# EEA-sensors/parallel-gps

Hardware: AMD Instinct MI355X
Metric: timesteps/sec (filter+smooth+log-lik) (higher is better)
Workload: dtype f64; 1 GPU; c2: matern32 state-dim 2, N=2^20 steps per GPU (1048576 total), f64, irregular times, prior-sampled observations; steps_per_gpu=1048576, steps_total=1048576, state_dim=2, parallelism=1 GPU

## Files before the change

### parallel-gps_amd/csrc/pgps_core.hip

```cpp
#include <chrono>
#include <algorithm>
#include <cmath>
#include <cstdlib>
#include <vector>
#include <cstdio>
#include <cstring>
#include <new>

#include "pgps_internal.h"
#include "pgps_gradlti.h"
#include "pgps_wc_args.h"

using namespace pgps;

namespace pgps {
int ensure(pgps_ctx* ctx, DevBuf& b, size_t bytes) {
    if (&b == &ctx->ws) ++ctx->ws_epoch;
    if (bytes <= b.cap) return PGPS_OK;
    if (b.p) HIPCHK(ctx, hipFree(b.p));
    b.p = nullptr;
    b.cap = 0;
    size_t want = bytes + bytes / 8 + 256;
    hipError_t e = hipMalloc(&b.p, want);
    if (e != hipSuccess) {
// ... 1048 lines not shown
template <typename T>
static int seg_smoother(pgps_ctx* ctx, long N, int d, int rank, int nranks, const T* Fs, const T* Qs, const T* fms,
                        const T* fPs, const T* gathered_s, T* sms, T* sPs, double* ll) {
    ScanArgs<T> a{};
    TRY(seg_common<T>(ctx, N, d, rank, nranks, a));
    if (!Fs || !Qs || !fms || !fPs || !gathered_s || !sms || !sPs) return PGPS_E_INVALID;
    if (!aligned16(Fs) || !aligned16(Qs) || !aligned16(fms) || !aligned16(fPs) || !aligned16(sms) ||
        !aligned16(sPs) || !aligned16(gathered_s))
        return PGPS_E_INVALID;
    a.Fs = Fs; a.Qs = Qs; a.fms = const_cast<T*>(fms); a.fPs = const_cast<T*>(fPs);
    a.gathered_s = gathered_s; a.sms = sms; a.sPs = sPs; a.ll = ll;
    if (!seg_follows(ctx, 3, N, d, rank, nranks)) return PGPS_E_INVALID;
    ctx->seg_tag.phase = 0;
    return dispatch_scan<T>(ctx, d, a, MODE_SEG_SMOOTHER);
}

#define PGPS_DEFINE_SEG(SUF, T)                                                                                      \
    extern "C" int pgps_seg_filter_reduce_dev_##SUF(pgps_ctx* c, long N, int d, int rank, int nranks, const T* P0,   \
                                                    const T* Fs, const T* Qs, const T* H, T R, const T* ys,         \
                                                    T* rec_f) {                                                     \
        return seg_reduce<T>(c, N, d, rank, nranks, P0, Fs, Qs, H, R, ys, rec_f);                                   \
    }                                                                                                                \
    extern "C" int pgps_seg_filter_apply_dev_##SUF(pgps_ctx* c, long N, int d, int rank, int nranks, const T* P0,    \
                                                   const T* Fs, const T* Qs, const T* H, T R, const T* ys,          \
                                                   const T* gathered_f, T* fms, T* fPs, T* rec_s) {                 \
        return seg_filter<T>(c, N, d, rank, nranks, P0, Fs, Qs, H, R, ys, gathered_f, fms, fPs, rec_s);             \
    }                                                                                                                \
    extern "C" int pgps_seg_smoother_apply_dev_##SUF(pgps_ctx* c, long N, int d, int rank, int nranks, const T* Fs,  \
                                                     const T* Qs, const T* fms, const T* fPs, const T* gathered_s,  \
                                                     T* sms, T* sPs, double* ll) {                                  \
        return seg_smoother<T>(c, N, d, rank, nranks, Fs, Qs, fms, fPs, gathered_s, sms, sPs, ll);                  \
    }

PGPS_DEFINE_SEG(f64, double)
PGPS_DEFINE_SEG(f32, float)

template <typename T>
static int pkfs_seg_run(pgps_ctx* ctx, long N, int d, const T* P0, const T* Fs, const T* Qs, const T* H, T R, const T* ys,
                        T* fms, T* fPs, T* sms, T* sPs, double* ll) {
    RoctxRange range_("parallel_filter");
    const int rank = ctx->comm_rank, nranks = ctx->comm_nranks;
    const size_t rf = ((size_t)seg_rec_f_len(d) * sizeof(T) + 15) / 16 * 16, rs = ((size_t)seg_rec_s_len(d) * sizeof(T) + 15) / 16 * 16;
    TRY(ensure(ctx, ctx->comm_buf, (rf + rs) * (size_t)(nranks + 1)));
    char* base = (char*)ctx->comm_buf.p;
    T* rec_f = (T*)base;
    T* rec_s = (T*)(base + rf);
    T* gat_f = (T*)(base + rf + rs);
    T* gat_s = (T*)(base + rf + rs + rf * (size_t)nranks);
    TRY(seg_reduce<T>(ctx, N, d, rank, nranks, P0, Fs, Qs, H, R, ys, rec_f));
    TRY(comm_allgather(ctx, rec_f, gat_f, (size_t)seg_rec_f_len(d) * sizeof(T)));
    TRY(seg_filter<T>(ctx, N, d, rank, nranks, P0, Fs, Qs, H, R, ys, gat_f, fms, fPs, rec_s));
    TRY(comm_allgather(ctx, rec_s, gat_s, (size_t)seg_rec_s_len(d) * sizeof(T)));
    return seg_smoother<T>(ctx, N, d, rank, nranks, Fs, Qs, fms, fPs, gat_s, sms, sPs, ll);
}

template <typename T>
static int pkfs_seg_dev(pgps_ctx* ctx, long N, int d, const T* P0, const T* Fs, const T* Qs, const T* H, T R, const T* ys,
                        T* fms, T* fPs, T* sms, T* sPs, double* ll) {
    if (!ctx || N < 1 || !P0 || !Fs || !Qs || !H || !ys || !fms || !fPs || !sms || !sPs) return PGPS_E_INVALID;
    if (!ctx->comm) return PGPS_E_INVALID;
    if (d < 1 || d > PGPS_MAX_DIM) return PGPS_E_UNSUPPORTED_DIM;
    return pkfs_seg_run<T>(ctx, N, d, P0, Fs, Qs, H, R, ys, fms, fPs, sms, sPs, ll);
}

extern "C" int pgps_pkfs_seg_dev_f64(pgps_ctx* c, long N, int d, const double* P0, const double* Fs, const double* Qs,
                                     const double* H, double R, const double* ys, double* fms, double* fPs, double* sms,
                                     double* sPs, double* ll) {
    return pkfs_seg_dev<double>(c, N, d, P0, Fs, Qs, H, R, ys, fms, fPs, sms, sPs, ll);
}
extern "C" int pgps_pkfs_seg_dev_f32(pgps_ctx* c, long N, int d, const float* P0, const float* Fs, const float* Qs,
                                     const float* H, float R, const float* ys, float* fms, float* fPs, float* sms, float* sPs,
                                     double* ll) {
    return pkfs_seg_dev<float>(c, N, d, P0, Fs, Qs, H, R, ys, fms, fPs, sms, sPs, ll);
}

template <typename T>
static int gp_dev(pgps_ctx* ctx, long N, int d, double lam, const double* N1, const double* N2, const double* Pinf,
                  const double* H, double R, const T* ts, double t0, const T* ys, T* fms, T* fPs, T* sms, T* sPs,
                  double* ll) {
    RoctxRange range_("parallel_filter");
    if (!ctx || N < 1 || !N1 || !Pinf || !H || !ts || !ys) return PGPS_E_INVALID;
    if (d < 1 || d > 3) return PGPS_E_UNSUPPORTED_DIM;
    if ((fms == nullptr) != (fPs == nullptr) || (sms == nullptr) != (sPs == nullptr)) return PGPS_E_INVALID;
    if (sms && !fms) return PGPS_E_INVALID;
    if (!fms && !ll) return PGPS_E_INVALID;
    if ((fms && (!aligned16(fms) || !aligned16(fPs))) || (sms && (!aligned16(sms) || !aligned16(sPs))))
        return PGPS_E_INVALID;
    GpArgs<T> g{};
    g.s.N = N;
    g.s.R = (T)R;
    g.s.ys = ys;
    g.s.fms = fms; g.s.fPs = fPs; g.s.sms = sms; g.s.sPs = sPs; g.s.ll = ll;
    g.m.lam = lam;
    for (int i = 0; i < 9; ++i) { g.m.N1[i] = 0; g.m.N2[i] = 0; g.m.Pinf[i] = 0; }
    for (int i = 0; i < d * d; ++i) { g.m.N1[i] = N1[i]; g.m.N2[i] = N2 ? N2[i] : 0.0; g.m.Pinf[i] = Pinf[i]; }
    for (int i = 0; i < 3; ++i) g.m.H[i] = i < d ? (T)H[i] : T(0);
    g.m.ts = ts;
    g.m.t_prev = (T)t0;
    if constexpr (sizeof(T) == 8) {
        if (resident_fits(ctx, N, d, false) && aligned16(ts) && aligned16(ys)) {
            ResArgs<double> ra{};
            ra.s = g.s;
            ra.m = g.m;
            return launch_resident<double, 2>(ctx, ra, true, sms != nullptr);
        }
    }
    switch (d) {
        case 1: return launch_gp<T, 1>(ctx, g, fms != nullptr, sms != nullptr);
        case 2: return launch_gp<T, 2>(ctx, g, fms != nullptr, sms != nullptr);
        case 3: return launch_gp<T, 3>(ctx, g, fms != nullptr, sms != nullptr);
        default: return PGPS_E_UNSUPPORTED_DIM;
    }
}

static int gp_adj_dev(pgps_ctx* ctx, long N, int d, double lam, const double* N1, const double* N2, const double* Pinf,
                      const double* H, double R, const double* ts, double t0, const double* ys, double* out) {
    RoctxRange range_("parallel_filter");
    if (!ctx || N < 1 || !N1 || !Pinf || !H || !ts || !ys || !out) return PGPS_E_INVALID;
    if (d < 1 || d > 3) return PGPS_E_UNSUPPORTED_DIM;
    GpArgs<double> g{};
    g.s.N = N;
    g.s.R = R;
    g.s.ys = ys;
    g.m.lam = lam;
    for (int i = 0; i < 9; ++i) { g.m.N1[i] = 0; g.m.N2[i] = 0; g.m.Pinf[i] = 0; }
    for (int i = 0; i < d * d; ++i) { g.m.N1[i] = N1[i]; g.m.N2[i] = N2 ? N2[i] : 0.0; g.m.Pinf[i] = Pinf[i]; }
    for (int i = 0; i < 3; ++i) g.m.H[i] = i < d ? H[i] : 0.0;
    g.m.ts = ts;
    g.m.t_prev = t0;
    switch (d) {
        case 1: return launch_gp_adj<double, 1>(ctx, g, out);
        case 2: return launch_gp_adj<double, 2>(ctx, g, out);
        case 3: return launch_gp_adj<double, 3>(ctx, g, out);
        default: return PGPS_E_UNSUPPORTED_DIM;
    }
}

extern "C" int pgps_gp_ll_grad_adj_dev_f64(pgps_ctx* ctx, long N, int d, double lam, const double* N1, const double* N2,
                                           const double* Pinf, const double* H, double R, const double* ts, double t0,
                                           const double* ys, double* out) {
    return gp_adj_dev(ctx, N, d, lam, N1, N2, Pinf, H, R, ts, t0, ys, out);
}

template <typename T>
static int gp_host(pgps_ctx* ctx, long N, int d, double lam, const double* N1, const double* N2, const double* Pinf,
                   const double* H, double R, const T* ts, double t0, const T* ys, T* fms, T* fPs, T* sms, T* sPs,
                   double* ll) {
    if (!ctx || N < 1 || !ts || !ys) return PGPS_E_INVALID;
    if (d < 1 || d > 3) return PGPS_E_UNSUPPORTED_DIM;
    HIPCHK(ctx, hipSetDevice(ctx->device));
    const size_t n = (size_t)N, dd = (size_t)d * d;
    const bool wf = fms || fPs || sms || sPs, wsm = sms || sPs;
    if (!wf) {
        SmallStage st(ctx, 2 * SmallStage::up(n * sizeof(T)), 16);
        if (st.ok) {
            double llh = 0.0;
            T* dys_ = st.in(ys, n);
            T* dts_ = st.in(ts, n);
            double* dll_ = st.out(&llh, 1);
            TRY(st.send());
            TRY(gp_dev<T>(ctx, N, d, lam, N1, N2, Pinf, H, R, dts_, t0, dys_, nullptr, nullptr, nullptr, nullptr, dll_));
            TRY(st.finish());
            if (ll) *ll = llh;
            return std::isfinite(llh) ? PGPS_OK : PGPS_E_NUMERIC;
        }
    }
    T *dts, *dys, *dfms = nullptr, *dfPs = nullptr, *dsms = nullptr, *dsPs = nullptr;
    double* dll;
    TRY(stage_in(ctx, ctx->st[4], ys, n, &dys));
    TRY(stage_in(ctx, ctx->st[10], ts, n, &dts));
    if (wf) {
        TRY(stage_in<T>(ctx, ctx->st[5], nullptr, n * d, &dfms));
        TRY(stage_in<T>(ctx, ctx->st[6], nullptr, n * dd, &dfPs));
    }
    if (wsm) {
        TRY(stage_in<T>(ctx, ctx->st[7], nullptr, n * d, &dsms));
        TRY(stage_in<T>(ctx, ctx->st[8], nullptr, n * dd, &dsPs));
    }
    TRY(stage_in<double>(ctx, ctx->st[9], nullptr, 2, &dll));
    TRY(gp_dev<T>(ctx, N, d, lam, N1, N2, Pinf, H, R, dts, t0, dys, dfms, dfPs, dsms, dsPs, dll));
    if (fms) TRY(stage_out(ctx, fms, dfms, n * d));
    if (fPs) TRY(stage_out(ctx, fPs, dfPs, n * dd));
    if (sms) TRY(stage_out(ctx, sms, dsms, n * d));
    if (sPs) TRY(stage_out(ctx, sPs, dsPs, n * dd));
    double llh = 0.0;
    TRY(stage_out(ctx, &llh, dll, 1));
    HIPCHK(ctx, hipStreamSynchronize(ctx->stream));
    if (ll) *ll = llh;
    if (!std::isfinite(llh)) return PGPS_E_NUMERIC;
// ... 1775 lines not shown
```

### parallel-gps_amd/csrc/pgps_resident.hip.h

```cpp
#pragma once

#include <type_traits>

#include "pgps_fused.hip.h"
#include "pgps_kernels.hip.h"

namespace pgps {


template <typename T, int D, int LC>
struct ResCfg {
    static constexpr int W = (int)sizeof(T), MAT = D * D, G = 4;
    static_assert(LC % G == 0, "whole sub-tiles");
    static constexpr int S = LC / G;
    using GF = StageGeom<MAT * W, G>;
    using GM = StageGeom<D * W, G>;
    static constexpr int SLOT = LC * MAT * W + 16;
    static constexpr int SLOTS = kWave * SLOT;
    static constexpr int MST = GM::BYTES > 5120 ? GM::BYTES : 5120;
    static constexpr int NSCAN = kWaves * Dim<D>::NFILT * W;
    static constexpr int BYTES = kWaves * (SLOTS + MST) + NSCAN + kWaves * 8;
};

__device__ __forceinline__ void res_wave_sync() {
    __builtin_amdgcn_fence(__ATOMIC_RELEASE, "wavefront");
    __builtin_amdgcn_wave_barrier();
    __builtin_amdgcn_fence(__ATOMIC_ACQUIRE, "wavefront");
}

template <typename T> struct ResForget;
template <> struct ResForget<double> { static constexpr double kA = 0x1p-120; };
template <> struct ResForget<float> { static constexpr float kA = 0x1p-60f; };

#define PGPS_RSTAMP(IDX)                                                                              \
    do {                                                                                              \
        if (ra.stamps && threadIdx.x == 0) ra.stamps[(long)blockIdx.x * 16 + (IDX)] = __builtin_readcyclecounter(); \
    } while (0)
#define PGPS_RSTAMP_WAVE(K)                                                                           \
    do {                                                                                              \
        if (ra.stamps && lane == 0)                                                                   \
            ra.stamps[(long)gridDim.x * 16 + (long)blockIdx.x * 8 + (K) * kWaves + wave] = __builtin_readcyclecounter(); \
    } while (0)

template <typename T>
__device__ __forceinline__ void res_skew(const ResArgs<T>& ra, int tile, int phase) {
    if (tile == ra.delay_tile && phase == ra.delay_phase) {
        const long long t0 = wall_clock64();
        ra.wstamps[(long)tile * 16 + 12] = t0;
        ra.wstamps[(long)tile * 16 + 13] = ra.delay_ticks;
        while (wall_clock64() - t0 < ra.delay_ticks) __builtin_amdgcn_s_sleep(8);
    }
}
template <typename T>
__device__ __forceinline__ void res_wstamp(const ResArgs<T>& ra, int tile, int slot) {
    if (ra.wstamps) ra.wstamps[(long)tile * 16 + slot] = wall_clock64();
}

template <typename T, int D>
__device__ __forceinline__ V4 res_pad_piece(int kind, int pos_in_rec) {
    constexpr int PER = 16 / (int)sizeof(T);
    T tmp[PER];
#pragma unroll
    for (int j = 0; j < PER; ++j) {
        const int e = (pos_in_rec * PER + j) % (D * D);
        tmp[j] = (kind == 0 && (e / D) == (e % D)) ? T(1) : T(0);
    }
    V4 v;
    __builtin_memcpy(&v, tmp, 16);
    return v;
}

template <typename T, int D, typename GEO, int PITCH>
__device__ __forceinline__ void res_issue(const char* __restrict__ g , int sb, long lim, bool full, int kind, V4* r) {
    const int lane = threadIdx.x & (kWave - 1);
    constexpr int NV = GEO::NV, OPI = kWave / NV;
    constexpr int PPR = D * D * (int)sizeof(T) / 16 > 0 ? D * D * (int)sizeof(T) / 16 : 1;
    const unsigned loff = (unsigned)(lane / NV) * PITCH + (unsigned)(lane % NV) * 16u;
    if (full) {
#pragma unroll
        for (int v = 0; v < NV; ++v) r[v] = *reinterpret_cast<const V4*>(g + ((long)sb * GEO::SEG + (long)v * OPI * PITCH) + loff);
    } else {
#pragma unroll
        for (int v = 0; v < NV; ++v) {
            const long off = (long)sb * GEO::SEG + (long)v * OPI * PITCH + loff;
            if (off < lim) r[v] = *reinterpret_cast<const V4*>(g + off);
            else r[v] = res_pad_piece<T, D>(kind, (lane % NV) % PPR);
        }
    }
}
template <typename GEO, int SLOT>
__device__ __forceinline__ void res_commit(char* slots, int sb, const V4* r) {
    const int lane = threadIdx.x & (kWave - 1);
    constexpr int NV = GEO::NV, OPI = kWave / NV;
    char* base = slots + (lane / NV) * SLOT + (lane % NV) * 16;
#pragma unroll
    for (int v = 0; v < NV; ++v) *reinterpret_cast<V4*>(base + sb * GEO::SEG + v * OPI * SLOT) = r[v];
}
template <typename GEO, int SLOT, int PITCH>
__device__ __forceinline__ void res_drain(char* __restrict__ g , int sb, long lim, bool full, const char* slots) {
    const int lane = threadIdx.x & (kWave - 1);
    constexpr int NV = GEO::NV, OPI = kWave / NV;
    const char* base = slots + (lane / NV) * SLOT + (lane % NV) * 16;
    const unsigned loff = (unsigned)(lane / NV) * PITCH + (unsigned)(lane % NV) * 16u;
#pragma unroll
    for (int v = 0; v < NV; ++v) {
        const V4 x = *reinterpret_cast<const V4*>(base + sb * GEO::SEG + v * OPI * SLOT);
        const long off = (long)sb * GEO::SEG + (long)v * OPI * PITCH + loff;
        if (full || off < lim) *reinterpret_cast<V4*>(g + ((long)sb * GEO::SEG + (long)v * OPI * PITCH) + loff) = x;
    }
}
template <typename GEO, int PITCH>
__device__ __forceinline__ void res_drain_m(char* __restrict__ g , int sb, long lim, bool full, const char* mst) {
    const int lane = threadIdx.x & (kWave - 1);
    constexpr int NV = GEO::NV, OPI = kWave / NV;
    const char* base = mst + (lane / NV) * GEO::STRIDE + (lane % NV) * 16;
    const unsigned loff = (unsigned)(lane / NV) * PITCH + (unsigned)(lane % NV) * 16u;
#pragma unroll
    for (int v = 0; v < NV; ++v) {
        const V4 x = *reinterpret_cast<const V4*>(base + v * OPI * GEO::STRIDE);
        const long off = (long)sb * GEO::SEG + (long)v * OPI * PITCH + loff;
        if (full || off < lim) *reinterpret_cast<V4*>(g + ((long)sb * GEO::SEG + (long)v * OPI * PITCH) + loff) = x;
    }
}

__device__ __forceinline__ void res_wait_all(int* bar, int nblocks, int* status) {
    if (threadIdx.x < 8) {
        const int want = (nblocks - (int)threadIdx.x + 7) / 8;
        if (want > 0) wait_flag(bar + threadIdx.x * 32, want, status);
    }
    __syncthreads();
}
__device__ __forceinline__ void res_arrive(int* bar, int tile) {
    __hip_atomic_fetch_add(bar + (tile & 7) * 32, 1, __ATOMIC_RELAXED, __HIP_MEMORY_SCOPE_AGENT);
}

__device__ __forceinline__ bool res_wait_epoch(const int* f, int want, int* status) {
    int spins = 0;
    while (__hip_atomic_load(f, __ATOMIC_RELAXED, __HIP_MEMORY_SCOPE_AGENT) != want) {
        __builtin_amdgcn_s_sleep(2);
        if (++spins > (1 << 22)) {
            atomicOr(status, 2);
            return false;
        }
    }
    return true;
}

template <typename T, int D>
__device__ __forceinline__ void res_filt_extend(FiltElem<T, D>& e, const T* F, const T* Q , T y, const T* h, T R) {
    T Ap[D * D], bp[D], FC[D * D], Cp[Dim<D>::SYM];
    mat_mul<T, D>(F, e.A, Ap);
    mat_vec<T, D>(F, e.b, bp);
    predict_cov<T, D>(F, e.C, Q, FC, Cp);
    const bool obs = !is_nan(y);
    T u[D], v[D];
    sym_vec<T, D>(Cp, h, u);
    mat_t_vec<T, D>(Ap, h, v);
    T S = R, hb = T(0);
#pragma unroll
    for (int i = 0; i < D; ++i) { S += h[i] * u[i]; hb += h[i] * bp[i]; }
    const T inv = obs ? recip(S) : T(0);
    const T res = obs ? y - hb : T(0);
#pragma unroll
    for (int i = 0; i < D; ++i) {
        const T Ki = u[i] * inv;
#pragma unroll
        for (int j = 0; j < D; ++j) e.A[i * D + j] = Ap[i * D + j] - Ki * v[j];
        e.b[i] = bp[i] + Ki * res;
        e.eta[i] += v[i] * (res * inv);
    }
#pragma unroll
    for (int i = 0; i < D; ++i)
#pragma unroll
        for (int j = i; j < D; ++j) {
            e.C[symi<D>(i, j)] = Cp[symi<D>(i, j)] - u[i] * u[j] * inv;
            e.J[symi<D>(i, j)] += v[i] * v[j] * inv;
        }
}

template <typename T, int D>
__device__ __forceinline__ void res_kf_step(MeanCov<T, D>& s, const T* F, const T* Q , T y, const T* h, T R, LogLik& ll,
                                            T* mp, T* Pp, T* FP) {
    mat_vec<T, D>(F, s.m, mp);
    predict_cov<T, D>(F, s.P, Q, FP, Pp);
    const bool obs = !is_nan(y);
    T u[D];
    sym_vec<T, D>(Pp, h, u);
    T S = R, mu = T(0);
#pragma unroll
    for (int i = 0; i < D; ++i) { S += h[i] * u[i]; mu += h[i] * mp[i]; }
    const T rinv = recip(S);
    {
        const double r = obs ? ll_diff(y, mu) : 0.0;
        const double Sw = obs ? ll_wide(S) : 1.0;
        ll.quad += r * r * (obs ? double(rinv) : 0.0);
        int e;
        ll.mant = std::frexp(ll.mant * Sw, &e);
        ll.expo += e;
        ll.count += obs ? 1 : 0;
    }
    const T inv = obs ? rinv : T(0);
    const T res = obs ? y - mu : T(0);
#pragma unroll
    for (int i = 0; i < D; ++i) s.m[i] = mp[i] + u[i] * (res * inv);
// ... 156 lines not shown
__device__ __forceinline__ void res_block_reduce_ordered(const E& mine, E& total, typename ElemTraits<E>::Scalar* lds) {
    using TR = ElemTraits<E>;
    const int lane = threadIdx.x & (kWave - 1);
    const int wave = __builtin_amdgcn_readfirstlane((int)(threadIdx.x / kWave));
    E acc = mine;
    res_wave_scan_inclusive<E, true>(acc, lane);
    if (lane == kWave - 1) rec_store(lds + wave * TR::N, acc);
    __syncthreads();
    E t;
    TR::identity(t);
    if (lane < kWaves) rec_load(lds + lane * TR::N, t);
    res_scan4<E, true>(t, lane);
    total = res_readlane_elem(t, kWaves - 1);
    __syncthreads();
}

template <typename T, int LC>
struct ResLaneValues {
    using GY = StageGeom<64, 1>;
    static constexpr int PER = 64 / (int)sizeof(T);
    static constexpr int R = LC / PER > 0 ? LC / PER : 1;
    static_assert(LC % PER == 0, "whole rounds");
    V4 r[R][GY::NV];
    __device__ __forceinline__ void issue(const T* __restrict__ g ) {
        const int lane = threadIdx.x & (kWave - 1);
        constexpr int NV = GY::NV, OPI = kWave / NV, PITCH = LC * (int)sizeof(T);
        const unsigned loff = (unsigned)(lane / NV) * PITCH + (unsigned)(lane % NV) * 16u;
#pragma unroll
        for (int rd = 0; rd < R; ++rd)
#pragma unroll
            for (int v = 0; v < NV; ++v)
                r[rd][v] = *reinterpret_cast<const V4*>(reinterpret_cast<const char*>(g) + ((long)rd * 64 + (long)v * OPI * PITCH) + loff);
    }
    __device__ __forceinline__ void finish(char* mst, T* out) {
        const int lane = threadIdx.x & (kWave - 1);
#pragma unroll
        for (int rd = 0; rd < R; ++rd) {
            res_wave_sync();
            constexpr int NV = GY::NV, OPI = kWave / NV;
            char* base = mst + (lane / NV) * GY::STRIDE + (lane % NV) * 16;
#pragma unroll
            for (int v = 0; v < NV; ++v) *reinterpret_cast<V4*>(base + v * OPI * GY::STRIDE) = r[rd][v];
            res_wave_sync();
            load_rec<T, PER>(reinterpret_cast<const T*>(mst + lane * GY::STRIDE), out + rd * PER);
        }
        res_wave_sync();
    }
};

template <typename T, int D, int LC, bool FUSED, bool SMOOTH = true, bool SKEW = false>
__global__ __launch_bounds__(kBlock) void k_pkfs_resident(const ResArgs<T> ra) {
    using CFG = ResCfg<T, D, LC>;
    using GF = typename CFG::GF;
    using GM = typename CFG::GM;
    using FE = FiltElem<T, D>;
    using SE = SmthElem<T, D>;
    using MC = MeanCov<T, D>;
    constexpr int MAT = D * D, SYM = Dim<D>::SYM, NF = Dim<D>::NFILT, NS = Dim<D>::NSMTH, G = CFG::G, S = CFG::S;
    constexpr int SLOT = CFG::SLOT;
    static_assert(kBlock == 256, "one workgroup of four waves per CU");
    static_assert(D <= 2, "resident pass: d <= 2");
    const ScanArgs<T>& a = ra.s;

    __shared__ __attribute__((aligned(16))) char smem[CFG::BYTES];
    const int tile = blockIdx.x;
    const int lane = threadIdx.x & (kWave - 1);
    const int wave = __builtin_amdgcn_readfirstlane((int)(threadIdx.x / kWave));
    char* slots = smem + wave * CFG::SLOTS;
    char* mst = smem + kWaves * CFG::SLOTS + wave * CFG::MST;
    T* lds = reinterpret_cast<T*>(smem + kWaves * (CFG::SLOTS + CFG::MST));
    double* lds_ll = reinterpret_cast<double*>(smem + kWaves * (CFG::SLOTS + CFG::MST) + CFG::NSCAN);
    char* myslot = slots + lane * SLOT;
    T* myrec = reinterpret_cast<T*>(myslot);

    PGPS_RSTAMP(0);
    if (tile == 0 && threadIdx.x < 16) ra.bar_next[threadIdx.x * 32] = 0;

    const long N = a.N;
    const long gt = (long)tile * kBlock + threadIdx.x;
    const long k0 = gt * LC;
    const long wbase = ((long)tile * kBlock + wave * kWave) * LC;
    const bool full = (wbase + (long)kWave * LC <= N);
    constexpr int PF = LC * MAT * (int)sizeof(T), PM = LC * D * (int)sizeof(T);
    const long limF = (N - wbase) * MAT * (long)sizeof(T), limM = (N - wbase) * D * (long)sizeof(T);

    T h[D], P0[SYM];
    if constexpr (FUSED) {
        gp_prior<T, D>(ra.m, h, P0);
    } else {
        T P0f[MAT];
#pragma unroll
        for (int i = 0; i < MAT; ++i) P0f[i] = a.P0[i];
        sym_from_full<T, D>(P0f, P0);
#pragma unroll
        for (int i = 0; i < D; ++i) h[i] = a.H[i];
    }
    const T Rn = a.R;

    T Freg[LC][MAT];
    T yreg[LC];
    constexpr int GL = MAT - SYM;
    static_assert(D - GL == 1, "one component of g per step stays in registers");
    FE agg;
    filt_identity(agg);
    auto reduce_step = [&](int j, const T* Qf) {
        T Q[SYM];
        sym_from_full<T, D>(Qf, Q);
        if (j == 0) {
            if (k0 == 0) filt_first(agg, P0, yreg[0], h, Rn);
            else res_filt_extend(agg, Freg[0], Q, yreg[0], h, Rn);
        } else {
            res_filt_extend(agg, Freg[j], Q, yreg[j], h, Rn);
        }
    };
    {
        const T nanv = T(__builtin_nan(""));
        if constexpr (FUSED) {
            T tv[LC];
            const T* tp = ra.m.ts;
            T tprev;
            if (full) {
                ResLaneValues<T, LC> lt, ly;
                lt.issue(tp + wbase);
                ly.issue(a.ys + wbase);
                lt.finish(mst, tv);
                ly.finish(mst, yreg);
                tprev = wshfl_up(tv[LC - 1], 1);
                if (lane == 0) tprev = (k0 > 0) ? tp[k0 - 1] : ra.m.t_prev;
            } else {
                const T tl = tp[N - 1];
#pragma unroll
                for (int j = 0; j < LC; ++j) {
                    const bool in = k0 + j < N;
                    tv[j] = in ? tp[in ? k0 + j : 0] : tl;
                    yreg[j] = in ? a.ys[in ? k0 + j : 0] : nanv;
                }
                tprev = (k0 > 0) ? (k0 - 1 < N ? tp[k0 - 1 < N ? k0 - 1 : 0] : tl) : ra.m.t_prev;
            }
#pragma unroll
            for (int j = 0; j < LC; ++j) {
                T Qf[MAT];
                lti_step<T, D>(ra.m, tv[j] - tprev, Freg[j], Qf);
                tprev = tv[j];
                store_rec<T, MAT>(myrec + j * MAT, Qf);
                reduce_step(j, Qf);
            }
        } else {
            const char* gF = reinterpret_cast<const char*>(a.Fs + wbase * MAT);
            const char* gQ = reinterpret_cast<const char*>(a.Qs + wbase * MAT);
            auto stream = [&](auto full_tag) {
                constexpr bool FULL = decltype(full_tag)::value;
                V4 rF[2][GF::NV], rQ[2][GF::NV];
                ResLaneValues<T, LC> ly;
                if constexpr (FULL) ly.issue(a.ys + wbase);
                res_issue<T, D, GF, PF>(gF, 0, limF, FULL, 0, rF[0]);
                res_issue<T, D, GF, PF>(gQ, 0, limF, FULL, 1, rQ[0]);
                if (S > 1) {
                    res_issue<T, D, GF, PF>(gF, 1, limF, FULL, 0, rF[1]);
                    res_issue<T, D, GF, PF>(gQ, 1, limF, FULL, 1, rQ[1]);
                }
                if constexpr (FULL) {
                    ly.finish(mst, yreg);
                } else {
#pragma unroll
                    for (int j = 0; j < LC; ++j) yreg[j] = (k0 + j < N) ? a.ys[k0 + j < N ? k0 + j : 0] : nanv;
                }
#pragma unroll
// ... 34 lines not shown
        asm volatile("s_waitcnt vmcnt(0)" ::: "memory");
        pub_store(ra.flags1 + tile, ra.epoch);
        if constexpr (SKEW) res_wstamp(ra, tile, 10);
        res_arrive(ra.bar, tile);
    });
    PGPS_RSTAMP(2);

    MC s;
#pragma unroll
    for (int i = 0; i < D; ++i) s.m[i] = T(0);
#pragma unroll
    for (int i = 0; i < SYM; ++i) s.P[i] = P0[i];
    bool waited_all = false;
    if (tile > 0) {
        if (a.shortcut != 0) {
            if (threadIdx.x == 0) res_wait_epoch(ra.flags1 + tile - 1, ra.epoch, a.status);
            __syncthreads();
        } else {
            res_wait_all(ra.bar, a.nblocks, a.status);
            waited_all = true;
        }
        FE nb;
        {
            T v[NF];
#pragma unroll
            for (int i = 0; i < NF; ++i) v[i] = pub_load(a.spine + (long)(tile - 1) * NF + i);
            unpack(v, nb);
        }
        T amax = T(0);
#pragma unroll
        for (int i = 0; i < MAT; ++i) amax = fmax(amax, fabs(nb.A[i]));
        const bool forget = a.shortcut != 0 && amax <= ResForget<T>::kA;
        if (__builtin_amdgcn_readfirstlane((int)forget)) {
#pragma unroll
            for (int i = 0; i < D; ++i) s.m[i] = nb.b[i];
#pragma unroll
            for (int i = 0; i < SYM; ++i) s.P[i] = nb.C[i];
        } else {
            if (!waited_all) res_wait_all(ra.bar, a.nblocks, a.status);
            FE mine, left;
            filt_identity(mine);
            if ((int)threadIdx.x < tile) {
                T v[NF];
                const T* rec = reinterpret_cast<const T*>(reinterpret_cast<const char*>(a.spine) + threadIdx.x * (unsigned)(NF * sizeof(T)));
#pragma unroll
                for (int i = 0; i < NF; ++i) v[i] = pub_load(rec + i);
                unpack(v, mine);
            }
            res_block_reduce_ordered(mine, left, lds);
            filt_apply(s, left);
        }
    }
    PGPS_RSTAMP(3);
    filt_apply(s, excl);
    PGPS_RSTAMP(4);

    LogLik ll;
    SE sagg;
    smth_identity(sagg);
    T Fh[MAT], Qh[MAT];
    T Qn[MAT];
    load_rec<T, MAT>(myrec, Qn);
    if constexpr (SMOOTH) {
#pragma unroll
        for (int i = 0; i < MAT; ++i) {
            Fh[i] = wshfl_down(Freg[0][i], 1);
            Qh[i] = wshfl_down(Qn[i], 1);
        }
        if (lane == kWave - 1) {
            const long k1 = k0 + LC;
            if (k1 < N) {
                if constexpr (FUSED) {
                    lti_step<T, D>(ra.m, ra.m.ts[k1] - ra.m.ts[k1 - 1], Fh, Qh);
                } else {
                    load_rec<T, MAT>(a.Fs + k1 * MAT, Fh);
                    load_rec<T, MAT>(a.Qs + k1 * MAT, Qh);
                }
            } else {
#pragma unroll
                for (int i = 0; i < MAT; ++i) { Fh[i] = (i / D == i % D) ? T(1) : T(0); Qh[i] = T(0); }
            }
        }
    }
    auto element = [&](long k_next, const MC& prev, const T* mp, const T* Pp, T* FP, SE& e) {
        const bool last = (k_next == N);
#pragma unroll
        for (int q = 0; q < MAT; ++q) FP[q] = last ? T(0) : FP[q];
        smth_element(prev, mp, Pp, FP, e);
    };
    const bool store_f = (a.fms != nullptr);
    char* gP = reinterpret_cast<char*>(a.fPs + wbase * MAT);
    char* gM = reinterpret_cast<char*>(a.fms + wbase * D);
    T Lhold[MAT];
#pragma unroll
    for (int sb = 0; sb < S; ++sb) {
        T Lnew[G][MAT];
#pragma unroll
        for (int i = 0; i < G; ++i) {
            const int j = sb * G + i;
            T Q[SYM];
            sym_from_full<T, D>(Qn, Q);
#ifndef PGPS_RES_NOQPF
            if (j + 1 < LC) load_rec<T, MAT>(myrec + (j + 1) * MAT, Qn);
#endif
#ifdef PGPS_RES_NOQPF
            if (j + 1 < LC) load_rec<T, MAT>(myrec + (j + 1) * MAT, Qn);
#endif
            MC prev = s;
            T mp[D], Pp[SYM], FP[MAT];
            if (j == 0) {
                if (k0 == 0) kf_step(s, Freg[0], Q, yreg[0], h, Rn, true, ll, mp, Pp, FP);
                else res_kf_step(s, Freg[0], Q, yreg[0], h, Rn, ll, mp, Pp, FP);
            } else {
#ifndef PGPS_RES_BRANCHFREE
                kf_step(s, Freg[j], Q, yreg[j], h, Rn, false, ll, mp, Pp, FP);
#else
                res_kf_step(s, Freg[j], Q, yreg[j], h, Rn, ll, mp, Pp, FP);
#endif
                if constexpr (SMOOTH) {
                    SE e, r;
                    element(k0 + j, prev, mp, Pp, FP, e);
                    smth_combine(sagg, e, r);
                    sagg = r;
#pragma unroll
                    for (int q = 0; q < MAT; ++q) Freg[j - 1][q] = e.E[q];
                    yreg[j - 1] = e.g[D - 1];
#pragma unroll
                    for (int q = 0; q < MAT; ++q) {
                        const T x = q < SYM ? e.L[q < SYM ? q : 0] : e.g[q < SYM ? 0 : q - SYM];
                        if (i == 0) Lhold[q] = x; else Lnew[i - 1][q] = x;
                    }
                }
            }
            T Pf[MAT];
            full_from_sym<T, D>(s.P, Pf);
            store_rec<T, MAT>(myrec + j * MAT, Pf);
            store_rec<T, D>(reinterpret_cast<T*>(mst + lane * GM::STRIDE) + i * D, s.m);
#ifndef PGPS_RES_NOSB
            __builtin_amdgcn_sched_barrier(0);
#endif
        }
        res_wave_sync();
        if (store_f) {
            res_drain<GF, SLOT, PF>(gP, sb, limF, full, slots);
            res_drain_m<GM, PM>(gM, sb, limM, full, mst);
        }
        res_wave_sync();
        if constexpr (SMOOTH) {
            if (sb > 0) store_rec<T, MAT>(myrec + (sb * G - 1) * MAT, Lhold);
#pragma unroll
            for (int i = 0; i + 1 < G; ++i) store_rec<T, MAT>(myrec + (sb * G + i) * MAT, Lnew[i]);
        }
    }
    if constexpr (!SMOOTH) {
        PGPS_RSTAMP_WAVE(1);
        PGPS_RSTAMP(5);
        const double v = ll.value();
        const double t = block_sum_double(v, lds_ll);
        if (threadIdx.x == 0) {
            if constexpr (SKEW) res_skew(ra, tile, 2);
            pub_store(a.llpart + tile, t);
            asm volatile("s_waitcnt vmcnt(0)" ::: "memory");
            if constexpr (SKEW) res_wstamp(ra, tile, 11);
            res_arrive(ra.bar2, tile);
        }
        if (tile == 0 && a.ll != nullptr) {
            res_wait_all(ra.bar2, a.nblocks, a.status);
            double w = 0.0;
            for (int b = threadIdx.x; b < a.nblocks; b += kBlock) w += pub_load(a.llpart + b);
            const double tt = block_sum_double(w, lds_ll);
            if (threadIdx.x == 0) *a.ll = tt;
        }
        PGPS_RSTAMP(9);
        return;
    }
    {
        constexpr int j = LC - 1;
        T Q[SYM], mp[D], Pp[SYM], FP[MAT];
        sym_from_full<T, D>(Qh, Q);
        mat_vec<T, D>(Fh, s.m, mp);
        predict_cov<T, D>(Fh, s.P, Q, FP, Pp);
        SE e, r;
        element(k0 + LC, s, mp, Pp, FP, e);
        smth_combine(sagg, e, r);
        sagg = r;
#pragma unroll
        for (int q = 0; q < MAT; ++q) Freg[j][q] = e.E[q];
        yreg[j] = e.g[D - 1];
        T Lg[MAT];
#pragma unroll
        for (int q = 0; q < MAT; ++q) Lg[q] = q < SYM ? e.L[q < SYM ? q : 0] : e.g[q < SYM ? 0 : q - SYM];
        store_rec<T, MAT>(myrec + j * MAT, Lg);
    }
    PGPS_RSTAMP_WAVE(1);
    PGPS_RSTAMP(5);
    SE sexcl;
    res_block_scan_exclusive<SE, false>(sagg, sexcl, lds, [&](const SE& stotal) {
        T vv[NS];
        pack(stotal, vv);
        if constexpr (SKEW) res_skew(ra, tile, 2);
#pragma unroll
        for (int i = 0; i < NS; ++i) pub_store(a.sspine + (long)tile * NS + i, vv[i]);
        asm volatile("s_waitcnt vmcnt(0)" ::: "memory");
        pub_store(ra.flags2 + tile, ra.epoch);
    });
    PGPS_RSTAMP(6);
    {
        const double v = ll.value();
        const double t = block_sum_double(v, lds_ll);
        if (threadIdx.x == 0) {
            pub_store(a.llpart + tile, t);
            asm volatile("s_waitcnt vmcnt(0)" ::: "memory");
            if constexpr (SKEW) res_wstamp(ra, tile, 11);
            res_arrive(ra.bar2, tile);
        }
    }

#pragma unroll
    for (int i = 0; i < D; ++i) s.m[i] = T(0);
#pragma unroll
    for (int i = 0; i < SYM; ++i) s.P[i] = T(0);
    waited_all = false;
    if (tile + 1 < a.nblocks) {
        if (a.shortcut != 0) {
            if (threadIdx.x == 0) res_wait_epoch(ra.flags2 + tile + 1, ra.epoch, a.status);
            __syncthreads();
        } else {
            res_wait_all(ra.bar2, a.nblocks, a.status);
            waited_all = true;
        }
        SE nb;
        {
            T v[NS];
#pragma unroll
            for (int i = 0; i < NS; ++i) v[i] = pub_load(a.sspine + (long)(tile + 1) * NS + i);
            unpack(v, nb);
        }
        T emax = T(0);
#pragma unroll
        for (int i = 0; i < MAT; ++i) emax = fmax(emax, fabs(nb.E[i]));
        const bool forget = a.shortcut != 0 && emax <= ResForget<T>::kA;
        if (__builtin_amdgcn_readfirstlane((int)forget)) {
#pragma unroll
            for (int i = 0; i < D; ++i) s.m[i] = nb.g[i];
#pragma unroll
            for (int i = 0; i < SYM; ++i) s.P[i] = nb.L[i];
        } else {
            if (!waited_all) { res_wait_all(ra.bar2, a.nblocks, a.status); waited_all = true; }
            SE mine, right;
            smth_identity(mine);
            const int b = tile + 1 + (int)threadIdx.x;
            if (b < a.nblocks) {
                T v[NS];
                const T* rec = reinterpret_cast<const T*>(reinterpret_cast<const char*>(a.sspine + (long)(tile + 1) * NS) +
                                                          threadIdx.x * (unsigned)(NS * sizeof(T)));
#pragma unroll
                for (int i = 0; i < NS; ++i) v[i] = pub_load(rec + i);
                unpack(v, mine);
            }
            res_block_reduce_ordered(mine, right, lds);
            smth_apply(right, s);
        }
    }
    PGPS_RSTAMP(7);
    smth_apply(sexcl, s);
    PGPS_RSTAMP(8);
    if (tile == 0 && a.ll != nullptr) {
        if (!waited_all) res_wait_all(ra.bar2, a.nblocks, a.status);
        double v = 0.0;
        for (int b = threadIdx.x; b < a.nblocks; b += kBlock) v += pub_load(a.llpart + b);
        const double t = block_sum_double(v, lds_ll);
        if (threadIdx.x == 0) *a.ll = t;
    }
    char* oP = reinterpret_cast<char*>(a.sPs + wbase * MAT);
    char* oM = reinterpret_cast<char*>(a.sms + wbase * D);
    T Ln[MAT];
    load_rec<T, MAT>(myrec + (LC - 1) * MAT, Ln);
#pragma unroll
    for (int sb = S - 1; sb >= 0; --sb) {
#pragma unroll
        for (int i = G - 1; i >= 0; --i) {
            const int j = sb * G + i;
            SE e;
#pragma unroll
            for (int q = 0; q < MAT; ++q) e.E[q] = Freg[j][q];
            e.g[D - 1] = yreg[j];
#pragma unroll
            for (int q = 0; q < SYM; ++q) e.L[q] = Ln[q];
#pragma unroll
            for (int q = SYM; q < MAT; ++q) e.g[q - SYM] = Ln[q];
            if (j > 0) load_rec<T, MAT>(myrec + (j - 1) * MAT, Ln);
            smth_apply(e, s);
            T Pf[MAT];
            full_from_sym<T, D>(s.P, Pf);
            store_rec<T, MAT>(myrec + j * MAT, Pf);
            store_rec<T, D>(reinterpret_cast<T*>(mst + lane * GM::STRIDE) + i * D, s.m);
        }
        res_wave_sync();
        res_drain<GF, SLOT, PF>(oP, sb, limF, full, slots);
        res_drain_m<GM, PM>(oM, sb, limM, full, mst);
        res_wave_sync();
    }
    PGPS_RSTAMP(9);
}

}
```

Baseline: 22.57 billion timesteps/s.

## Interleave filtered covariance drains with next sub-tile compute in resident kernel

The drain of filtered covariances from LDS slots to global memory is deferred by one sub-tile and split into pieces issued inside the per-step compute loop, so global stores overlap the filter arithmetic. The smoother's L records are held in registers an extra sub-tile (Lwait) so they don't overwrite slots that are still draining. Bounds checks switch to 32-bit offsets, and element() compares a local index instead of a long global index. The gp_dev validation now lets smoothing without filtered outputs reach the resident path. The cost is higher register pressure from Lwait and more complex ordering around LDS reuse.

```diff
diff --git a/parallel-gps_amd/csrc/pgps_core.hip b/parallel-gps_amd/csrc/pgps_core.hip
--- a/parallel-gps_amd/csrc/pgps_core.hip
+++ b/parallel-gps_amd/csrc/pgps_core.hip
@@ -1154,8 +1154,7 @@
     if (!ctx || N < 1 || !N1 || !Pinf || !H || !ts || !ys) return PGPS_E_INVALID;
     if (d < 1 || d > 3) return PGPS_E_UNSUPPORTED_DIM;
     if ((fms == nullptr) != (fPs == nullptr) || (sms == nullptr) != (sPs == nullptr)) return PGPS_E_INVALID;
-    if (sms && !fms) return PGPS_E_INVALID;
-    if (!fms && !ll) return PGPS_E_INVALID;
+    if (!fms && !sms && !ll) return PGPS_E_INVALID;
     if ((fms && (!aligned16(fms) || !aligned16(fPs))) || (sms && (!aligned16(sms) || !aligned16(sPs))))
         return PGPS_E_INVALID;
     GpArgs<T> g{};
@@ -1177,6 +1176,7 @@
             return launch_resident<double, 2>(ctx, ra, true, sms != nullptr);
         }
     }
+    if (sms && !fms) return PGPS_E_INVALID;
     switch (d) {
         case 1: return launch_gp<T, 1>(ctx, g, fms != nullptr, sms != nullptr);
         case 2: return launch_gp<T, 2>(ctx, g, fms != nullptr, sms != nullptr);
diff --git a/parallel-gps_amd/csrc/pgps_resident.hip.h b/parallel-gps_amd/csrc/pgps_resident.hip.h
--- a/parallel-gps_amd/csrc/pgps_resident.hip.h
+++ b/parallel-gps_amd/csrc/pgps_resident.hip.h
@@ -96,30 +96,55 @@
 #pragma unroll
     for (int v = 0; v < NV; ++v) *reinterpret_cast<V4*>(base + sb * GEO::SEG + v * OPI * SLOT) = r[v];
 }
+__device__ __forceinline__ int res_lim32(long lim) { return lim < 0 ? 0 : (lim > (1L << 30) ? (1 << 30) : (int)lim); }
 template <typename GEO, int SLOT, int PITCH>
-__device__ __forceinline__ void res_drain(char* __restrict__ g , int sb, long lim, bool full, const char* slots) {
+__device__ __forceinline__ void res_drain_part(char* __restrict__ g , int sb, int v0, int nv, int lim, bool full,
+                                               const char* slots) {
     const int lane = threadIdx.x & (kWave - 1);
     constexpr int NV = GEO::NV, OPI = kWave / NV;
     const char* base = slots + (lane / NV) * SLOT + (lane % NV) * 16;
     const unsigned loff = (unsigned)(lane / NV) * PITCH + (unsigned)(lane % NV) * 16u;
-#pragma unroll
-    for (int v = 0; v < NV; ++v) {
-        const V4 x = *reinterpret_cast<const V4*>(base + sb * GEO::SEG + v * OPI * SLOT);
-        const long off = (long)sb * GEO::SEG + (long)v * OPI * PITCH + loff;
-        if (full || off < lim) *reinterpret_cast<V4*>(g + ((long)sb * GEO::SEG + (long)v * OPI * PITCH) + loff) = x;
-    }
+    if (full) {
+        V4 x[NV];
+#pragma unroll
+        for (int v = 0; v < NV; ++v)
+            if (v >= v0 && v < v0 + nv) x[v] = *reinterpret_cast<const V4*>(base + sb * GEO::SEG + v * OPI * SLOT);
+#pragma unroll
+        for (int v = 0; v < NV; ++v)
+            if (v >= v0 && v < v0 + nv) *reinterpret_cast<V4*>(g + ((long)sb * GEO::SEG + (long)v * OPI * PITCH) + loff) = x[v];
+    } else {
+#pragma unroll
+        for (int v = 0; v < NV; ++v) {
+            if (v < v0 || v >= v0 + nv) continue;
+            const V4 x = *reinterpret_cast<const V4*>(base + sb * GEO::SEG + v * OPI * SLOT);
+            if ((int)loff < lim - (sb * GEO::SEG + v * OPI * PITCH))
+                *reinterpret_cast<V4*>(g + ((long)sb * GEO::SEG + (long)v * OPI * PITCH) + loff) = x;
+        }
+    }
+}
+template <typename GEO, int SLOT, int PITCH>
+__device__ __forceinline__ void res_drain(char* __restrict__ g , int sb, int lim, bool full, const char* slots) {
+    res_drain_part<GEO, SLOT, PITCH>(g, sb, 0, GEO::NV, lim, full, slots);
 }
 template <typename GEO, int PITCH>
-__device__ __forceinline__ void res_drain_m(char* __restrict__ g , int sb, long lim, bool full, const char* mst) {
+__device__ __forceinline__ void res_drain_m(char* __restrict__ g , int sb, int lim, bool full, const char* mst) {
     const int lane = threadIdx.x & (kWave - 1);
     constexpr int NV = GEO::NV, OPI = kWave / NV;
     const char* base = mst + (lane / NV) * GEO::STRIDE + (lane % NV) * 16;
     const unsigned loff = (unsigned)(lane / NV) * PITCH + (unsigned)(lane % NV) * 16u;
-#pragma unroll
-    for (int v = 0; v < NV; ++v) {
-        const V4 x = *reinterpret_cast<const V4*>(base + v * OPI * GEO::STRIDE);
-        const long off = (long)sb * GEO::SEG + (long)v * OPI * PITCH + loff;
-        if (full || off < lim) *reinterpret_cast<V4*>(g + ((long)sb * GEO::SEG + (long)v * OPI * PITCH) + loff) = x;
+    if (full) {
+        V4 x[NV];
+#pragma unroll
+        for (int v = 0; v < NV; ++v) x[v] = *reinterpret_cast<const V4*>(base + v * OPI * GEO::STRIDE);
+#pragma unroll
+        for (int v = 0; v < NV; ++v) *reinterpret_cast<V4*>(g + ((long)sb * GEO::SEG + (long)v * OPI * PITCH) + loff) = x[v];
+    } else {
+#pragma unroll
+        for (int v = 0; v < NV; ++v) {
+            const V4 x = *reinterpret_cast<const V4*>(base + v * OPI * GEO::STRIDE);
+            if ((int)loff < lim - (sb * GEO::SEG + v * OPI * PITCH))
+                *reinterpret_cast<V4*>(g + ((long)sb * GEO::SEG + (long)v * OPI * PITCH) + loff) = x;
+        }
     }
 }
 
@@ -442,7 +467,8 @@
     const long wbase = ((long)tile * kBlock + wave * kWave) * LC;
     const bool full = (wbase + (long)kWave * LC <= N);
     constexpr int PF = LC * MAT * (int)sizeof(T), PM = LC * D * (int)sizeof(T);
-    const long limF = (N - wbase) * MAT * (long)sizeof(T), limM = (N - wbase) * D * (long)sizeof(T);
+    const long limF = (N - wbase) * MAT * (long)sizeof(T);
+    const int limP = res_lim32(limF), limM = res_lim32((N - wbase) * D * (long)sizeof(T));
 
     T h[D], P0[SYM];
     if constexpr (FUSED) {
@@ -643,8 +669,9 @@
             }
         }
     }
-    auto element = [&](long k_next, const MC& prev, const T* mp, const T* Pp, T* FP, SE& e) {
-        const bool last = (k_next == N);
+    const int to_end = (N - k0 < 0) ? -1 : (N - k0 > LC ? LC + 1 : (int)(N - k0));
+    auto element = [&](int j_next, const MC& prev, const T* mp, const T* Pp, T* FP, SE& e) {
+        const bool last = (j_next == to_end);
 #pragma unroll
         for (int q = 0; q < MAT; ++q) FP[q] = last ? T(0) : FP[q];
         smth_element(prev, mp, Pp, FP, e);
@@ -652,21 +679,18 @@
     const bool store_f = (a.fms != nullptr);
     char* gP = reinterpret_cast<char*>(a.fPs + wbase * MAT);
     char* gM = reinterpret_cast<char*>(a.fms + wbase * D);
+    constexpr int NVP = GF::NV, PPS = (NVP + G - 2) / (G - 1);
     T Lhold[MAT];
+    T Lwait[G - 1][MAT];
 #pragma unroll
     for (int sb = 0; sb < S; ++sb) {
-        T Lnew[G][MAT];
+        T Lnew[G - 1][MAT];
 #pragma unroll
         for (int i = 0; i < G; ++i) {
             const int j = sb * G + i;
             T Q[SYM];
             sym_from_full<T, D>(Qn, Q);
-#ifndef PGPS_RES_NOQPF
             if (j + 1 < LC) load_rec<T, MAT>(myrec + (j + 1) * MAT, Qn);
-#endif
-#ifdef PGPS_RES_NOQPF
-            if (j + 1 < LC) load_rec<T, MAT>(myrec + (j + 1) * MAT, Qn);
-#endif
             MC prev = s;
             T mp[D], Pp[SYM], FP[MAT];
             if (j == 0) {
@@ -680,7 +704,7 @@
 #endif
                 if constexpr (SMOOTH) {
                     SE e, r;
-                    element(k0 + j, prev, mp, Pp, FP, e);
+                    element(j, prev, mp, Pp, FP, e);
                     smth_combine(sagg, e, r);
                     sagg = r;
 #pragma unroll
@@ -697,23 +721,28 @@
             full_from_sym<T, D>(s.P, Pf);
             store_rec<T, MAT>(myrec + j * MAT, Pf);
             store_rec<T, D>(reinterpret_cast<T*>(mst + lane * GM::STRIDE) + i * D, s.m);
+            if (sb > 0 && store_f) res_drain_part<GF, SLOT, PF>(gP, sb - 1, i * PPS, PPS, limP, full, slots);
 #ifndef PGPS_RES_NOSB
             __builtin_amdgcn_sched_barrier(0);
 #endif
         }
         res_wave_sync();
-        if (store_f) {
-            res_drain<GF, SLOT, PF>(gP, sb, limF, full, slots);
-            res_drain_m<GM, PM>(gM, sb, limM, full, mst);
-        }
+        if (store_f) res_drain_m<GM, PM>(gM, sb, limM, full, mst);
         res_wave_sync();
         if constexpr (SMOOTH) {
-            if (sb > 0) store_rec<T, MAT>(myrec + (sb * G - 1) * MAT, Lhold);
-#pragma unroll
-            for (int i = 0; i + 1 < G; ++i) store_rec<T, MAT>(myrec + (sb * G + i) * MAT, Lnew[i]);
+            if (sb > 0) {
+#pragma unroll
+                for (int i = 0; i + 1 < G; ++i) store_rec<T, MAT>(myrec + ((sb - 1) * G + i) * MAT, Lwait[i]);
+                store_rec<T, MAT>(myrec + (sb * G - 1) * MAT, Lhold);
+            }
+#pragma unroll
+            for (int i = 0; i + 1 < G; ++i)
+#pragma unroll
+                for (int q = 0; q < MAT; ++q) Lwait[i][q] = Lnew[i][q];
         }
     }
     if constexpr (!SMOOTH) {
+        if (store_f) res_drain_part<GF, SLOT, PF>(gP, S - 1, 0, NVP, limP, full, slots);
         PGPS_RSTAMP_WAVE(1);
         PGPS_RSTAMP(5);
         const double v = ll.value();
@@ -736,13 +765,14 @@
         return;
     }
     {
+        if (store_f) res_drain_part<GF, SLOT, PF>(gP, S - 1, 0, NVP / 2, limP, full, slots);
         constexpr int j = LC - 1;
         T Q[SYM], mp[D], Pp[SYM], FP[MAT];
         sym_from_full<T, D>(Qh, Q);
         mat_vec<T, D>(Fh, s.m, mp);
         predict_cov<T, D>(Fh, s.P, Q, FP, Pp);
         SE e, r;
-        element(k0 + LC, s, mp, Pp, FP, e);
+        element(LC, s, mp, Pp, FP, e);
         smth_combine(sagg, e, r);
         sagg = r;
 #pragma unroll
@@ -751,6 +781,13 @@
         T Lg[MAT];
 #pragma unroll
         for (int q = 0; q < MAT; ++q) Lg[q] = q < SYM ? e.L[q < SYM ? q : 0] : e.g[q < SYM ? 0 : q - SYM];
+#pragma unroll
+        for (int q = 0; q < MAT; ++q) asm volatile("" : "+v"(Lg[q]));
+        __builtin_amdgcn_sched_barrier(0);
+        if (store_f) res_drain_part<GF, SLOT, PF>(gP, S - 1, NVP / 2, NVP - NVP / 2, limP, full, slots);
+        res_wave_sync();
+#pragma unroll
+        for (int i = 0; i + 1 < G; ++i) store_rec<T, MAT>(myrec + ((S - 1) * G + i) * MAT, Lwait[i]);
         store_rec<T, MAT>(myrec + j * MAT, Lg);
     }
     PGPS_RSTAMP_WAVE(1);
@@ -858,7 +895,7 @@
             store_rec<T, D>(reinterpret_cast<T*>(mst + lane * GM::STRIDE) + i * D, s.m);
         }
         res_wave_sync();
-        res_drain<GF, SLOT, PF>(oP, sb, limF, full, slots);
+        res_drain<GF, SLOT, PF>(oP, sb, limP, full, slots);
         res_drain_m<GM, PM>(oM, sb, limM, full, mst);
         res_wave_sync();
     }
```

Measured after the change: 23.45 billion timesteps/s, median of 6. 3.9% higher.
